# swami1995/SimuRLacra

Hardware: AMD Instinct MI355X
Metric: env-steps/sec whole node, 65 536 QQubeSwingUpSim envs, random policy (higher is better)
Workload: dtype f32

## Files before the change

scratch/ubench/rec_stream.hip:

```cpp
#include <hip/hip_runtime.h>
#include <cstdio>
#include <cstdlib>
typedef float v4f __attribute__((ext_vector_type(4)));
template <int LAYOUT, bool NT>
__global__ __launch_bounds__(256) void k(v4f* __restrict__ out, int n, int T, int pad, int jitter) {
    const int i = blockIdx.x * blockDim.x + threadIdx.x;
    const int wave = i >> 6, lane = i & 63;
    float x = (float)i * 1e-9f;
    const int mypad = pad + (jitter ? (wave * 2654435761u >> 16) % (unsigned)jitter : 0);
    for (int t = 0; t < T; ++t) {
        for (int q = 0; q < mypad; ++q) x = __builtin_fmaf(x, 0.999f, 1e-3f);
        v4f a = {x, x + 1.f, x + 2.f, x + 3.f}, b = {x + 4.f, x + 5.f, x + 6.f, x + 7.f};
        v4f *p0, *p1;
        if (LAYOUT == 0) {
            p0 = out + ((size_t)t * 2 + 0) * n + i;
            p1 = out + ((size_t)t * 2 + 1) * n + i;
        } else {
            p0 = out + (((size_t)wave * T + t) * 2 + 0) * 64 + lane;
            p1 = p0 + 64;
        }
        if (NT) {
            __builtin_nontemporal_store(a, p0);
            __builtin_nontemporal_store(b, p1);
        } else {
            *p0 = a;
            *p1 = b;
        }
    }
}
int main() {
    hipEvent_t e0, e1;
    hipEventCreate(&e0), hipEventCreate(&e1);
    const size_t cap = (size_t)6 << 30;
    v4f* buf;
    if (hipMalloc(&buf, cap) != hipSuccess) return 1;
    hipMemset(buf, 0, cap);
    const int ns[] = {65536, 131072, 262144, 1048576};
    const int pads[] = {0, 100, 200, 400};
    for (int n : ns)
        for (int wg : {64, 256})
            for (int pad : pads)
                for (int jit : {0, 64})
                    for (int layout = 0; layout < 2; ++layout)
                        for (int nt = 0; nt < 2; ++nt) {
                            size_t per_t = (size_t)n * 32;
                            int T = (int)((cap / 2) / per_t);
                            if (T > 400) T = 400;
                            float best = 1e30f;
                            for (int rep = 0; rep < 4; ++rep) {
                                v4f* o = buf + (rep & 1) * (cap / 2 / 16);
                                hipEventRecord(e0);
                                if (layout == 0 && nt == 0) k<0, false><<<n / wg, wg>>>(o, n, T, pad, jit);
                                if (layout == 0 && nt == 1) k<0, true><<<n / wg, wg>>>(o, n, T, pad, jit);
                                if (layout == 1 && nt == 0) k<1, false><<<n / wg, wg>>>(o, n, T, pad, jit);
                                if (layout == 1 && nt == 1) k<1, true><<<n / wg, wg>>>(o, n, T, pad, jit);
                                hipEventRecord(e1);
                                hipEventSynchronize(e1);
                                float ms;
                                hipEventElapsedTime(&ms, e0, e1);
                                if (rep && ms < best) best = ms;
                            }
                            printf("n=%8d wg=%3d pad=%3d jitter=%2d layout=%d nt=%d T=%3d : %7.1f us  %6.0f GB/s  %6.1f ns/step\n", n, wg, pad,
                                   jit, layout, nt, T, best * 1e3, per_t * T / best * 1e-6, best * 1e6 / T);
                            fflush(stdout);
                        }
    return 0;
}
```

simurlacra_amd/csrc/vecsim.hip:

```cpp
#include "vecsim_kernels.h"

namespace vs {

__global__ void k_bump_row(int* row) { *row += 1; }

__global__ __launch_bounds__(256) void k_rollout_lengths(const uint32_t* __restrict__ words, size_t ld, int n, int t_steps,
                                                         long long* __restrict__ lengths, uint8_t* __restrict__ done_last) {
    const int i = blockIdx.x * 256 + threadIdx.x;
    if (i >= n) return;
    const int nw = (t_steps + 31) / 32;
    int first = -1;
    for (int w = 0; w < nw && first < 0; ++w) {
        uint32_t bits = words[(size_t)w * ld + i];
        if (w == nw - 1 && (t_steps & 31)) bits &= (1u << (t_steps & 31)) - 1u;
        if (bits) first = w * 32 + (__ffs((int)bits) - 1);
    }
    lengths[i] = first < 0 ? (long long)t_steps : (long long)first + 1;
    done_last[i] = first >= 0;
}

__global__ void k_count_err(const uint8_t* err, int n, unsigned long long* out) {
    int i = blockIdx.x * BLOCK + threadIdx.x;
    bool e = i < n && err[i] != 0;
    unsigned long long m = __builtin_amdgcn_ballot_w64(e);
// ... 189 lines not shown
        out->s[q] = specs[q];
    }
    return VS_OK;
}

struct vs_mixed {
    int n = 0;
    vs_handle sub[MAX_SEG]{};
    Segs host{};
    Segs* dev = nullptr;
    int total_blocks = 0;
    std::string err;
};

static bool mixed_redraws(const vs_mixed* m) {
    for (int q = 0; q < m->n; ++q)
        if (m->sub[q]->d.dr_n > 0 || m->sub[q]->d.pbuf_n > 0) return true;
    return false;
}

static int mixed_upload(vs_mixed* m, const float* const* acts, const int64_t* env_strides, const int64_t* dim_strides,
                        int k_steps) {
    int blocks = 0;
    vs_handle h0 = m->sub[0];
    for (int q = 0; q < m->n; ++q) {
        vs_handle h = m->sub[q];
        if (h->d.pipe.act_on || h->d.pipe.obs_on) {
            m->err = "mixed batch: a segment carries an action/observation pipeline (single-family handles only)";
            return VS_ERR_STATE;
        }
        Seg& sg = m->host.s[q];
        blocks += (h->d.ld + BLOCK - 1) / BLOCK;
        sg.type = h->type;
        sg.block_end = blocks;
        sg.T = h->task;
        sg.d = h->d;
        sg.act = acts ? acts[q] : nullptr;
        sg.env_stride = env_strides ? (long)env_strides[q] : 0;
        sg.dim_stride = dim_strides ? (long)dim_strides[q] : 0;
        sg.reset_seed = h->ar_seed;
        sg.epoch0 = h->epoch;
        h->epoch += (uint64_t)k_steps;
    }
    m->host.n = m->n;
    m->total_blocks = blocks;
    hipError_t e = hipMemcpyAsync(m->dev, &m->host, sizeof(Segs), hipMemcpyHostToDevice, h0->stream);
    if (e == hipSuccess) e = hipStreamSynchronize(h0->stream);
    if (e != hipSuccess) { m->err = std::string("mixed_upload: ") + hipGetErrorString(e); return VS_ERR_HIP; }
    return VS_OK;
}

extern "C" {

int vs_version(void) { return 304; }

static int record_width(int t, int mode) {
    const EnvInfo& e = ENV_INFO[t];
    return mode == 2 ? e.O + e.A + 1 + e.S + e.A + e.H : e.O + e.A + 1;
}

int vs_traj_layout(int t, int mode, int* F, int* nq, int* h2, int* h1) {
    if (t < 0 || t >= VS_ENV_COUNT || mode < 1 || mode > 2) return VS_ERR_ARG;
    const int f = record_width(t, mode);
    if (F) *F = f;
    if (nq) *nq = f / 4;
    if (h2) *h2 = (f % 4) >= 2 ? 1 : 0;
    if (h1) *h1 = f % 2;
    return VS_OK;
}

int vs_env_dims(int t, int* S, int* A, int* O, int* P, int* H, int* I, int* K) {
    if (t < 0 || t >= VS_ENV_COUNT) return VS_ERR_ARG;
    const EnvInfo& e = ENV_INFO[t];
    if (S) *S = e.S;
    if (A) *A = e.A;
    if (O) *O = e.O;
    if (P) *P = e.P;
    if (H) *H = e.H;
    if (I) *I = e.I;
    if (K) *K = e.K;
    return VS_OK;
}

const char* vs_env_name(int t) { return (t < 0 || t >= VS_ENV_COUNT) ? nullptr : ENV_INFO[t].name; }

const char* vs_param_name(int t, int i) {
    if (t < 0 || t >= VS_ENV_COUNT || i < 0 || i >= ENV_INFO[t].P) return nullptr;
    return ENV_INFO[t].pnames[i];
}

int vs_nominal_params(int t, int flags, float* out) {
    if (t < 0 || t >= VS_ENV_COUNT || !out) return VS_ERR_ARG;
    for (int k = 0; k < ENV_INFO[t].P; ++k) out[k] = ENV_INFO[t].nominal[k];
    if ((t == VS_ENV_QCP_SU || t == VS_ENV_QCP_ST) && (flags & VS_FLAG_LONG_POLE)) {
        out[12] = 0.23f;
        out[13] = 0.641f / 2;
    }
    return VS_OK;
}

const char* vs_last_error(vs_handle h) { return h ? h->err.c_str() : g_create_err.c_str(); }

int vs_create(int env_type, int64_t n_envs, double dt, int64_t max_steps, int device_id, const vs_task_cfg* cfg,
              vs_handle* out) {
    if (!out) return fail(nullptr, VS_ERR_ARG, "vs_create: out is NULL");
    *out = nullptr;
    if (env_type < 0 || env_type >= VS_ENV_COUNT) return fail(nullptr, VS_ERR_ARG, "vs_create: unknown env_type");
// ... 840 lines not shown
```

simurlacra_amd/csrc/vecsim_envs.h:

```cpp
#pragma once
#include <hip/hip_runtime.h>
#include <stdint.h>

#include <type_traits>

#include "vecsim_dual.h"

namespace vs {

constexpr int MAXS = 8, MAXA = 2, MAXO = 8, MAXH = 2, MAXP = 20, MAXK = 20;
constexpr double PI_D = 3.14159265358979323846;
constexpr float PI_F = (float)PI_D;
constexpr float PI_4_F = (float)(PI_D / 4.0), PI4_F = (float)(4.0 * PI_D), PI5_F = (float)(5.0 * PI_D),
                PI20_F = (float)(20.0 * PI_D), QQ_TH_MAX_F = (float)(115.0 / 180.0 * PI_D);
constexpr float TWO_PI_F = 6.28318530717958647692f;
constexpr float TWO_PI_HI = 6.28318548202514648437500f;
constexpr float TWO_PI_LO = -1.74845553146951715461910e-07f;

enum RewKind { REW_QUADR = 0, REW_EXP = 1, REW_SCALED_EXP = 2 };

struct Task {
    float des[MAXS];
    float qd[MAXS];
    float rd[MAXA];
// ... 135 lines not shown
        }
        return c;
    }
    __device__ __forceinline__ static uint4 philox(uint64_t seed, uint32_t env, uint32_t purpose, uint64_t t) {
        return rounds(make_uint4(env, purpose, (uint32_t)t, (uint32_t)(t >> 32)),
                      make_uint2((uint32_t)seed, (uint32_t)(seed >> 32)));
    }
    __device__ __forceinline__ static float to_u01(uint32_t bits) { return (float)(bits >> 8) * (1.0f / 16777216.0f); }
    __device__ __forceinline__ void block() {
        out = rounds(ctr, key);
        ctr.y += 0x10000u;
        used = 0;
    }
    __device__ __forceinline__ uint32_t next() {
        if (used == 4) block();
        uint32_t v = used == 0 ? out.x : used == 1 ? out.y : used == 2 ? out.z : out.w;
        ++used;
        return v;
    }
    __device__ __forceinline__ float u01() { return to_u01(next()); }
    __device__ __forceinline__ float uniform(float lo, float hi) { return lo + (hi - lo) * u01(); }
    __device__ __forceinline__ static void box_muller(uint32_t b0, uint32_t b1, float& z0, float& z1) {
        float u1 = 1.0f - to_u01(b0);
        float u2 = to_u01(b1);
        float r = __builtin_amdgcn_sqrtf(-1.3862944f * __builtin_amdgcn_logf(u1));
        z0 = r * __builtin_amdgcn_cosf(u2);
        z1 = r * __builtin_amdgcn_sinf(u2);
    }
    __device__ __forceinline__ float normal() {
        uint32_t b0 = next(), b1 = next();
        float z0, z1;
        box_muller(b0, b1, z0, z1);
        return z0;
    }
};
enum RngPurpose { RNG_ACT = 1, RNG_INIT = 2, RNG_PARAM = 3, RNG_ACT_NOISE = 4, RNG_OBS_NOISE = 5, RNG_POLICY_NOISE = 6 };

enum FinalKind { FINAL_NONE = 0, FINAL_CONST_MALUS = 1, FINAL_STATE_TIME = 2 };
template <int A_>
struct EnvDefaults {
    static constexpr bool SYMMETRIC_BOX = true;
    static constexpr int FINAL = FINAL_NONE;
    static constexpr bool WS_PAYS = true;
    static constexpr bool REWARD_SIDE_USES_CONSTS = true;
    static constexpr int WS_SHAPE_FULL = 64;
    static constexpr bool WS_MID = true;
    static constexpr int WS_MID_G3_FROM = 1 << 30;
    static constexpr int WS_SMALL = 64;
    static constexpr int WS_PREP_C = 0;
    static constexpr int WS_PREP_G64 = 0;
    static constexpr bool WS_DRAW_P = false;
    static constexpr bool WS_G3 = false;
    static constexpr int WS_G3_FULL = 256;
    static constexpr int WS_MIN_WAVES = 1;
    static constexpr bool WS_ALONE = false;
    template <class R>
    __device__ static void limit_act(const float*, const float* lo, const float* hi, const R* a_raw, R* a) {
#pragma unroll
        for (int j = 0; j < A_; ++j) {
            a[j] = vmin(vmax(a_raw[j], lo[j]), hi[j]);
            if (visnan(a_raw[j])) a[j] = a_raw[j];
        }
    }
    __device__ static float sample_action(const float*, float lo, float hi, float u01, int) { return lo + (hi - lo) * u01; }
    static constexpr int TRIG = 0, TRIG_AT = 0;
    template <class R>
    __device__ static void observe_p(const R*, R*) {}
};
#define VS_OBSERVE_C_IS_OBSERVE \
    template <class R>          \
    __device__ static void observe_c(const R* s, const R*, R* o) { observe(s, o); }

struct Omo : EnvDefaults<1> {
    static constexpr int WS_MID_G3_FROM = 0;
    static constexpr int WS_PREP_G64 = 1;
    static constexpr int S = 2, A = 1, O = 2, H = 0, I = 2, P = 3, K = 4, KS = 4;
    static constexpr int REW = REW_QUADR, RADIAL = -1, CMAX = -1;
    static constexpr int FINAL = FINAL_CONST_MALUS;
    static constexpr bool WS_DRAW_P = true;
    static constexpr bool WS_G3 = true;
    enum { C_A10, C_A11, C_B1, C_AMAX };
    __device__ static void calc_consts(const Task&, const float* p, float* c) {
        float m = p[0], k = p[1], d = p[2];
        float omega = sqrtf(k / m);
        float zeta = d / (2.0f * sqrtf(m * k));
        c[C_A10] = -(omega * omega);
        c[C_A11] = -2.0f * zeta * omega;
        c[C_B1] = 1.0f / m;
        c[C_AMAX] = 1.0f * k;
    }
    __device__ static void state_bounds(const float*, float* lo, float* hi) {
        hi[0] = 1.0f; hi[1] = 10.0f; lo[0] = -1.0f; lo[1] = -10.0f;
    }
    __device__ static void act_bounds(const float* c, float* lo, float* hi) { hi[0] = c[C_AMAX]; lo[0] = -c[C_AMAX]; }
    template <class R>
    __device__ static void dynamics(const Task& T, const float* c, R* s, R*, const R* a, const R*) {
        R sd0 = s[1];
        R sd1 = c[C_A10] * s[0] + c[C_A11] * s[1] + c[C_B1] * a[0];
        s[0] = s[0] + sd0 * T.dt;
        s[1] = s[1] + sd1 * T.dt;
    }
    template <class R>
    __device__ static void observe(const R* s, R* o) { o[0] = s[0]; o[1] = s[1]; }
    VS_OBSERVE_C_IS_OBSERVE
    __device__ static void sample_init(const Task&, const float*, Rng& g, float* init) {
        init[0] = g.uniform(-0.75f, -0.65f);
// ... 553 lines not shown
```

simurlacra_amd/csrc/vecsim_kernels.h:

```cpp
#pragma once
#include <hip/hip_runtime.h>

#include <climits>
#include <cmath>
#include <cstdio>
#include <cstdlib>
#include <cstring>
#include <new>
#include <string>
#include <type_traits>
#include <vector>

#include "../../include/vecsim.h"
#include "vecsim_envs.h"

namespace vs {

constexpr int BLOCK = 256;

struct DrSpecs {
    int n;
    vs_dp_spec s[MAXP];
};

// ... 689 lines not shown
            if (!UNI) E::act_bounds(c, alo, ahi);
        } else {
            if (fin) {
                es.count += 1u;
                es.retsum += ret;
                es.lensum += step;
            }
            if (d.log_episodes) append_episode(d, fin, i, ret, step);
            frozen |= done;
            if (!REC && __builtin_amdgcn_ballot_w64(!frozen) == 0ull) break;
        }
#ifdef VS_ABLATE_OBSERVE
        if (REC) { for (int j = 0; j < E::O; ++j) ob[j] = s[j % E::S]; }
#else
        if (REC) E::observe(s, ob);
#endif
    }
    i = VS_COLD(i);
    if (!REC) E::observe(s, ob);
    if (PIPE && d.pipe.obs_on) pipe_obs<E>(d, i, es.epi, step, ob, ob);
#pragma unroll
    for (int j = 0; j < E::S; ++j) d.state[j * ld + i] = s[j];
#pragma unroll
    for (int j = 0; j < E::H; ++j) d.hidden[j * ld + i] = h[j];
#pragma unroll
    for (int j = 0; j < E::O; ++j) d.obs[j * ld + i] = ob[j];
    d.step[i] = step;
    d.ret[i] = ret;
    d.rew[i] = rew;
    d.done[i] = done;
    d.failed[i] = failed;
    if (E::FINAL != FINAL_NONE) d.yielded[i] = yielded;
    d.ep_idx[i] = es.epi;
    d.es_count[i] = es.count;
    d.es_retsum[i] = es.retsum;
    d.es_lensum[i] = es.lensum;
}

template <class E, bool UNI, bool AR, int REC, bool PIPE, bool DRK = false>
__global__ __launch_bounds__(BLOCK) void k_rollout(Task T, Dev d, int k_steps, uint64_t seed, uint64_t reset_seed,
                                                   uint64_t epoch0) {
    rollout_body<E, UNI, AR, REC, PIPE, DRK>(T, d, k_steps, seed, reset_seed, epoch0, (int)blockIdx.x);
}

enum : unsigned { WSF_DONE = 1u, WSF_FAILED = 2u, WSF_FROZEN = 4u, WSF_FIN = 8u };

__device__ __forceinline__ void ws_barrier() {
#ifdef VS_WS_NOSYNC
    return;
#endif
    asm volatile("s_waitcnt lgkmcnt(0)\n\ts_barrier" ::: "memory");
}

constexpr int FNN_MAXH = 4;
constexpr int FNN_W = 64;
constexpr int FNN_XS = 12;
__host__ __device__ constexpr int fnn_waves(int n_hidden) { return n_hidden <= 2 ? 8 : 4; }
enum FnnNonlin { FNN_ID = 0, FNN_TANH = 1, FNN_RELU = 2, FNN_SIGMOID = 3 };
struct Fnn {
    const float* w;
    int n_hidden, in_dim, out_dim;
    int hidden[FNN_MAXH];
    int hid_nonlin[FNN_MAXH], out_nonlin;
    int feat;
    int n_vis;
    int obs_idx[MAXO];
    int ident;
    int noisy;
    float noise_std[MAXA];
    int off_w[FNN_MAXH + 1], off_b[FNN_MAXH + 1];
};

__device__ __forceinline__ float tanh_fast(float x) {
    float t = __builtin_amdgcn_exp2f(-2.885390081777927f * fabsf(x));
    float r = (1.0f - t) * rcp_fast(1.0f + t);
    return copysignf(r, x);
}
__device__ __forceinline__ float fnn_nonlin(int kind, float x) {
    if (kind == FNN_TANH) return tanh_fast(x);
    if (kind == FNN_RELU) return fmaxf(x, 0.f);
    if (kind == FNN_SIGMOID) return rcp_fast(1.0f + __builtin_amdgcn_exp2f(-1.4426950408889634f * x));
    return x;
}

__device__ __forceinline__ float wave_sum_to_lane63(float v) {
#define VS_DPP_ADD(ctrl, rmask)                                                                                             \
    v += __builtin_bit_cast(float, __builtin_amdgcn_update_dpp(0, __builtin_bit_cast(int, v), ctrl, rmask, 0xF, false))
    VS_DPP_ADD(0xB1, 0xF);
    VS_DPP_ADD(0x4E, 0xF);
    VS_DPP_ADD(0x141, 0xF);
    VS_DPP_ADD(0x140, 0xF);
    VS_DPP_ADD(0x142, 0xA);
    VS_DPP_ADD(0x143, 0xC);
#undef VS_DPP_ADD
    return v;
}

__device__ __forceinline__ void wave_lds_fence() {
    __builtin_amdgcn_fence(__ATOMIC_RELEASE, "wavefront");
    __builtin_amdgcn_wave_barrier();
    __builtin_amdgcn_fence(__ATOMIC_ACQUIRE, "wavefront");
}

typedef float fnn_acc __attribute__((ext_vector_type(16)));
template <class E, bool AR, int REC, int NHID, int NE, bool MF = false>
__global__ __launch_bounds__(64 * fnn_waves(NHID)) void k_rollout_fnn(Task T, Dev d, Fnn P, int k_steps, uint64_t reset_seed,
// ... 310 lines not shown
            auto_reset<E, UNI>(T, d, fin, i, reset_seed, c, s, h, step, ret, yielded, es);
            E::act_bounds(c, alo, ahi);
        } else {
            if (fin) {
                es.count += 1u;
                es.retsum += ret;
                es.lensum += step;
            }
            if (d.log_episodes) append_episode(d, fin, i, ret, step);
            frozen |= done;
        }
        E::observe(s, ob);
    }
    if (!envw) return;
#pragma unroll
    for (int j = 0; j < E::S; ++j) d.state[j * ld + i] = s[j];
#pragma unroll
    for (int j = 0; j < E::H; ++j) d.hidden[j * ld + i] = h[j];
#pragma unroll
    for (int j = 0; j < E::O; ++j) d.obs[j * ld + i] = ob[j];
    d.step[i] = step;
    d.ret[i] = ret;
    d.rew[i] = rew;
    d.done[i] = done;
    d.failed[i] = failed;
    if (E::FINAL != FINAL_NONE) d.yielded[i] = yielded;
    d.ep_idx[i] = es.epi;
    d.es_count[i] = es.count;
    d.es_retsum[i] = es.retsum;
    d.es_lensum[i] = es.lensum;
}

template <class E, bool UNI, bool AR, int REC, int WS_R, int NE, bool DP, int NR = 2, int DRK = 0>
__global__ __launch_bounds__(NR * NE)
__attribute__((amdgpu_waves_per_eu(NR == 3 ? 3 : E::WS_MIN_WAVES, (NE == 64 && NR == 2 && E::WS_ALONE) ? 1 : 0))) void k_rollout_ws(Task T, Dev d, int k_steps, uint64_t seed, uint64_t reset_seed,
                                                        uint64_t epoch0) {
    static_assert(DRK == 0 || (!UNI && AR), "a randomizer needs per-env constants and resets inside the launch");
    static_assert(DRK >= 0 && DRK <= 2, "none | randomizer | buffer");
    static_assert(E::FINAL != FINAL_STATE_TIME, "needs the post-step state on the reward side");
    static_assert(NE == 64 || NE == 128 || NE == 256, "envs per workgroup");
    static_assert(NR == 2 || (NR == 3 && !DP), "two roles, or three with the generator wave drawing the actions");
    constexpr bool G3 = NR == 3;
#ifdef VS_G_NOOBS
    constexpr bool GOBS = false;
#else
    constexpr bool GOBS = G3 && REC != 0 && E::O >= 4;
#endif
    constexpr int HM = REC == 2 ? E::H : 0;
    constexpr int AM = DP ? E::A : 0;
    constexpr int M0 = E::S + (REC ? E::TRIG : 0) + HM + AM + 1;
    constexpr int M = M0 % 4 == 3 ? M0 + 1 : M0;
    constexpr int TR0 = E::S, HM0 = E::S + (REC ? E::TRIG : 0), AM0 = HM0 + HM;
    constexpr int NT = E::TRIG > 0 ? E::TRIG : 1, NH = E::H > 0 ? E::H : 1;
    __shared__ __attribute__((aligned(16))) float l_msg[2][WS_R][M * NE];
#ifdef VS_PREP_G256
    constexpr int PCL = DP ? 0 : (E::WS_PREP_C > 0 ? E::WS_PREP_C : ((NR == 3 && DRK == 0) ? E::WS_PREP_G64 : 0));
#else
    constexpr int PCL = DP ? 0 : (E::WS_PREP_C > 0 ? E::WS_PREP_C : ((NR == 3 && NE == 64 && DRK == 0) ? E::WS_PREP_G64 : 0));
#endif
    constexpr bool PC = PCL > 0;
    static_assert(PCL != 2 || E::REWARD_SIDE_USES_CONSTS || DRK == 0, "a dead zone off the physics wave reads per-env constants: they must not change inside the launch");
    constexpr int AW = PC ? 2 * E::A : E::A;
    __shared__ __attribute__((aligned(16))) float l_act[G3 ? 3 : (DP ? 1 : 2)][DP ? 1 : WS_R][DP ? 4 : AW * NE];
    auto ab = [](int bb) __attribute__((always_inline)) { return DP ? 0 : (G3 ? bb % 3 : (bb & 1)); };
    constexpr bool STOCK = AR;
    constexpr int SKW = E::I + (REC ? E::TRIG : 0);
#ifdef VS_WS_REFILL
    constexpr int WS_REFILL = VS_WS_REFILL;
#else
    constexpr int WS_REFILL = 8;
#endif
    __shared__ float l_stock[STOCK ? SKW * NE : 1];
    __shared__ uint32_t l_stag[STOCK ? NE : 1];
    __shared__ uint32_t l_epi[(STOCK && G3) ? NE : 1];
    extern __shared__ float l_dyn[];
    const bool dr_stock = DRK == 1 ? (STOCK && !UNI && d.dr_n > 0) : (DRK == 2 && STOCK && !UNI && d.dr_n > 0 && d.pbuf_n == 0);
    const bool stock_on = STOCK && (DRK == 0 || (DRK == 1 ? true : (d.pbuf_n == 0 && (d.dr_n == 0 || dr_stock))));
    float* const l_npar = l_dyn;
    float* const l_ncon = l_dyn + E::P * NE;
    const int wave = threadIdx.x >> 6;
    const int role = wave / (NE / 64);
    const int le = threadIdx.x & (NE - 1);
    const int i = blockIdx.x * NE + le;
    const int le_ = le, i_ = i;
    const size_t ld = d.ld;
    const bool valid = i < d.n;
    const int nb = (k_steps + WS_R - 1) / WS_R;
    float c[E::K];
    load_consts<E, UNI>(d, i, c, 0, E::KS);
    float alo[E::A], ahi[E::A];
    E::act_bounds(c, alo, ahi);

    constexpr unsigned SPB = 4 / E::A;
    static_assert(WS_R % SPB == 0, "a batch is a whole number of Philox blocks");
    constexpr int NBLK = WS_R / SPB;
    const unsigned ph = (unsigned)(epoch0 % SPB);
    const uint64_t blk0 = epoch0 / SPB;
    uint4 carry = make_uint4(0, 0, 0, 0);
    auto draw_batch = [&](int bb, float (*a_out)[AW]) __attribute__((always_inline)) {
        uint32_t w[(NBLK + 1) * 4];
        w[0] = carry.x, w[1] = carry.y, w[2] = carry.z, w[3] = carry.w;
#pragma unroll
        for (int q = 1; q <= NBLK; ++q) {
            carry = Rng::philox(seed, d.idx0 + (uint32_t)i, RNG_ACT, blk0 + (uint64_t)bb * NBLK + (uint64_t)q);
            w[4 * q] = carry.x, w[4 * q + 1] = carry.y, w[4 * q + 2] = carry.z, w[4 * q + 3] = carry.w;
        }
#pragma unroll
        for (int r = 0; r < WS_R; ++r) {
#pragma unroll
            for (int j = 0; j < E::A; ++j) {
                uint32_t bits = w[r * E::A + j];
#pragma unroll
                for (unsigned p2 = 1; p2 < SPB; ++p2) bits = ph == p2 ? w[(r + p2) * E::A + j] : bits;
                bool nrm = (T.flags & VS_FLAG_ACT_NORM) != 0;
                a_out[r][(PC ? E::A : 0) + j] = E::sample_action(c, nrm ? -1.0f : alo[j], nrm ? 1.0f : ahi[j], Rng::to_u01(bits), j);
            }
            if constexpr (PC) {
                const float* a = a_out[r] + E::A;
                float an[E::A], ac[E::A];
                const bool nrm = (T.flags & VS_FLAG_ACT_NORM) != 0;
                float lb[E::A], ub[E::A];
                E::act_bounds(c, lb, ub);
#pragma unroll
                for (int j = 0; j < E::A; ++j) {
                    float m = lb[j] + (a[j] + 1.0f) * (ub[j] - lb[j]) * 0.5f;
                    an[j] = vsel(nrm, m, a[j]);
                }
                E::limit_act(c, alo, ahi, an, ac);
                if constexpr (PCL == 2) E::dead_zone(T, c, ac);
#pragma unroll
                for (int j = 0; j < E::A; ++j) a_out[r][j] = ac[j];
            }
        }
    };

    uint32_t c_epi = 0u;
    uint32_t c_tag = 0xFFFFFFFFu;
    auto refill = [&]() __attribute__((always_inline)) {
        if (!STOCK) return;
        if (G3) c_epi = __hip_atomic_load(&l_epi[le], __ATOMIC_RELAXED, __HIP_MEMORY_SCOPE_WORKGROUP);
        const bool need = stock_on && valid && c_tag != c_epi;
#ifdef VS_WS_REFILL_MIN
        constexpr int REFILL_MIN = DRK == 1 ? VS_WS_REFILL_MIN : 1;
#else
        constexpr int REFILL_MIN = DRK == 1 ? 8 : 1;
#endif
        if (__builtin_popcountll(__builtin_amdgcn_ballot_w64(need)) < REFILL_MIN) return;
        const int i = VS_COLD(i_), le = VS_COLD(le_);
        if (dr_stock) {
            Rng gp(reset_seed, d.idx0 + (uint32_t)i, RNG_PARAM, (uint64_t)c_epi);
            const int n = d.dr_n;
            for (int q = 0; q < n; ++q) {
                const vs_dp_spec sp = d.drv.s[q];
                const float v = draw_one_param(sp, gp);
                if (need) l_npar[sp.param_index * NE + le] = v;
            }
        }
        if (need) {
            float cs[E::K];
#pragma unroll
            for (int k = 0; k < E::K; ++k) cs[k] = k < E::KS ? c[k] : 0.f;
            if (dr_stock) {
                float p[E::P];
#pragma unroll
                for (int k = 0; k < E::P; ++k) p[k] = l_npar[k * NE + le];
                E::calc_consts(T, p, cs);
#pragma unroll
                for (int k = 0; k < E::K; ++k) l_ncon[k * NE + le] = cs[k];
            }
            Rng g(reset_seed, d.idx0 + (uint32_t)i, RNG_INIT, (uint64_t)c_epi);
            float init[E::I];
            E::sample_init(T, cs, g, init);
#pragma unroll
            for (int j = 0; j < E::I; ++j) l_stock[j * NE + le] = init[j];
            if (REC && E::TRIG > 0) {
                float s0[E::S], tr0[NT];
                E::state_from_init(init, s0);
                E::observe_p(s0, tr0);
#pragma unroll
                for (int j = 0; j < E::TRIG; ++j) l_stock[(E::I + j) * NE + le] = tr0[j];
            }
            __hip_atomic_store(&l_stag[le], c_epi, __ATOMIC_RELEASE, __HIP_MEMORY_SCOPE_WORKGROUP);
            c_tag = c_epi;
        }
    };
    auto draw = [&](int bb) __attribute__((always_inline)) {
        if (DP) return;
        float a_new[WS_R][AW];
        draw_batch(bb, a_new);
#pragma unroll
        for (int r = 0; r < WS_R; ++r) Planes<AW>::store(l_act[ab(bb)][DP ? 0 : r], NE, le, a_new[r]);
    };

    if (role == 0) {
        __builtin_amdgcn_s_setprio(3);
        float s[E::S], h[NH], tr[NT], ob[E::O];
#pragma unroll
        for (int j = 0; j < E::S; ++j) s[j] = d.state[j * ld + i];
#pragma unroll
        for (int j = 0; j < E::H; ++j) h[j] = d.hidden[j * ld + i];
        int step = d.step[i];
        uint32_t epi = d.ep_idx[i];
        bool frozen = !AR && d.done[i] != 0;
        bool done = d.done[i] != 0, failed = d.failed[i] != 0;
        bool err_acc = false;
        if (REC) E::observe_p(s, tr);
        if (DP) carry = Rng::philox(seed, d.idx0 + (uint32_t)i, RNG_ACT, blk0);
        __builtin_amdgcn_s_waitcnt(0x0F70);
        ws_barrier();
        auto p_step = [&](const float* a, float* msg) __attribute__((always_inline)) {
            {
                float v[M];
#pragma unroll
                for (int j = 0; j < E::S; ++j) v[j] = s[j];
                if (REC) {
#pragma unroll
                    for (int j = 0; j < E::TRIG; ++j) v[TR0 + j] = tr[j];
                }
#pragma unroll
                for (int j = 0; j < HM; ++j) v[HM0 + j] = h[j];
#pragma unroll
                for (int j = 0; j < AM; ++j) v[AM0 + j] = a[j];
                bool fin = false;
                if (!frozen) {
                    if constexpr (PCL == 2) {
                        E::dynamics_core(T, c, s, h, a, (REC && E::TRIG > 0) ? (const float*)tr : (const float*)nullptr);
                    } else if constexpr (PCL == 1) {
                        E::dynamics(T, c, s, h, a, (REC && E::TRIG > 0) ? (const float*)tr : (const float*)nullptr);
                    } else {
                        float an[E::A], ac[E::A];
                        {
                            const bool nrm = (T.flags & VS_FLAG_ACT_NORM) != 0;
                            float lb[E::A], ub[E::A];
                            E::act_bounds(c, lb, ub);
#pragma unroll
                            for (int j = 0; j < E::A; ++j) {
                                float m = lb[j] + (a[j] + 1.0f) * (ub[j] - lb[j]) * 0.5f;
                                an[j] = vsel(nrm, m, a[j]);
                            }
                        }
                        E::limit_act(c, alo, ahi, an, ac);
                        E::dynamics(T, c, s, h, ac, (REC && E::TRIG > 0) ? (const float*)tr : (const float*)nullptr);
// ... 24 lines not shown
#pragma unroll
                            for (int j = 0; j < E::S; ++j) err_acc |= isnan(s[j]);
                            load_consts<E, UNI>(d, i, c, E::KS, E::K);
                            bool stocked = false;
                            if (STOCK) {
                                const uint32_t tag = __hip_atomic_load(&l_stag[le], __ATOMIC_ACQUIRE, __HIP_MEMORY_SCOPE_WORKGROUP);
                                stocked = tag == epi;
                                if (stocked) {
                                    if (dr_stock) {
#pragma unroll
                                        for (int k = 0; k < E::K; ++k) c[k] = l_ncon[k * NE + le];
#pragma unroll
                                        for (int k = 0; k < E::P; ++k) d.params[(size_t)k * ld + i] = l_npar[k * NE + le];
#pragma unroll
                                        for (int k = 0; k < E::K; ++k) d.consts[(size_t)k * ld + i] = c[k];
                                    }
                                    float init[E::I];
#pragma unroll
                                    for (int j = 0; j < E::I; ++j) init[j] = l_stock[j * NE + le];
                                    if (REC) {
#pragma unroll
                                        for (int j = 0; j < E::TRIG; ++j) tr[j] = l_stock[(E::I + j) * NE + le];
                                    }
                                    E::state_from_init(init, s);
                                    E::init_hidden(T, c, nullptr, s, h, false);
                                }
                            }
#ifdef VS_WS_STAMP
                            if (d.dbg) atomicAdd(d.dbg + ((size_t)(i >> 6) * 3 + 0) * 4, stocked ? 1ull : (1ull << 32));
#endif
                            if (!stocked) {
                                reset_lane_sampled<E>(T, d, DRK != 0, i, reset_seed, (uint64_t)epi, c, s, h,
                                                      dr_stock ? (const float*)l_npar : (const float*)nullptr, NE, le, DRK == 2);
                                if (REC) E::observe_p(s, tr);
                            }
                            epi += 1u;
                            step = 0;
                            if (STOCK && G3) __hip_atomic_store(&l_epi[le], epi, __ATOMIC_RELEASE, __HIP_MEMORY_SCOPE_WORKGROUP);
                        }
                        if (!UNI) E::act_bounds(c, alo, ahi);
#ifdef VS_WS_STAMP
                        VS_STAMP(sr1);
                        if (d.dbg && (threadIdx.x & 63) == 0) {
                            atomicAdd(d.dbg + ((size_t)(i >> 6) * 3 + 2) * 4 + 0, sr1 - sr0);
                            atomicAdd(d.dbg + ((size_t)(i >> 6) * 3 + 2) * 4 + 1, 1ull);
                        }
#endif
                    }
                } else {
                    frozen |= done;
                }
            }
        };
        auto p_batch_full = [&](int b) __attribute__((always_inline)) {
            float a_all[WS_R][AW];
            if (DP) {
                draw_batch(b, a_all);
            } else {
#pragma unroll
                for (int r = 0; r < WS_R; ++r) Planes<AW>::load(l_act[ab(b)][DP ? 0 : r], NE, le, a_all[r]);
            }
#pragma unroll
            for (int r = 0; r < WS_R; ++r) p_step(a_all[r], l_msg[b & 1][r]);
        };
        auto p_batch_ragged = [&](int b, int nr) __attribute__((always_inline)) {
            float a_all[WS_R][AW];
            if (DP) draw_batch(b, a_all);
#pragma unroll 1
            for (int r = 0; r < nr; ++r) {
                float a[AW];
                if (DP) {
#pragma unroll
                    for (int j = 0; j < AW; ++j) {
                        a[j] = a_all[0][j];
#pragma unroll
                        for (int q = 1; q < WS_R; ++q) a[j] = r == q ? a_all[q][j] : a[j];
                    }
                } else {
                    Planes<AW>::load(l_act[ab(b)][DP ? 0 : r], NE, le, a);
                }
                p_step(a, l_msg[b & 1][r]);
            }
        };
#ifdef VS_WS_NOP
        for (int b = 0; b < nb; ++b) ws_barrier();
        if (false)
#endif
#ifdef VS_WS_STAMP
        unsigned long long acc0 = 0, acc1 = 0, acc2 = 0;
#endif
        for (int b = 0; b < nb; ++b) {
            const int nr = min(WS_R, k_steps - b * WS_R);
            VS_STAMP(st0);
            if (nr == WS_R) p_batch_full(b);
            else p_batch_ragged(b, nr);
            VS_STAMP(st2);
            ws_barrier();
#ifdef VS_WS_STAMP
            VS_STAMP(st3);
            acc1 += st2 - st0, acc2 += st3 - st2;
#endif
        }
#ifdef VS_WS_STAMP
        if ((threadIdx.x & 63) == 0 && d.dbg) {
            unsigned long long* q = d.dbg + ((size_t)(i >> 6) * 3 + 0) * 4;
            q[1] = acc1, q[2] = acc2, q[3] = (unsigned long long)nb;
        }
#endif
        const int i = VS_COLD(i_);
#pragma unroll
        for (int j = 0; j < E::S; ++j) err_acc |= isnan(s[j]);
        if (err_acc && valid) d.err[i] = 1;
        E::observe(s, ob);
#pragma unroll
        for (int j = 0; j < E::S; ++j) d.state[j * ld + i] = s[j];
#pragma unroll
        for (int j = 0; j < E::H; ++j) d.hidden[j * ld + i] = h[j];
#pragma unroll
        for (int j = 0; j < E::O; ++j) d.obs[j * ld + i] = ob[j];
        d.step[i] = step;
        d.ep_idx[i] = epi;
        d.done[i] = done;
        d.failed[i] = failed;
    } else if (role == 1) {
        const size_t rec0 = (size_t)d.traj_t0;
        float ret = d.ret[i];
        float rew = d.rew[i];
        bool yielded = E::FINAL != FINAL_NONE ? d.yielded[i] != 0 : false;
        EpStat es{0u, d.es_count[i], d.es_retsum[i], d.es_lensum[i]};
        int len = d.step[i];
        DoneBits db;
        if (REC) db.begin(d, i, rec0);
        if (STOCK && !G3) {
            c_epi = d.ep_idx[i];
            l_stag[le] = 0xFFFFFFFFu;
            if (dr_stock) {
#pragma unroll
                for (int k = 0; k < E::P; ++k) l_npar[k * NE + le] = d.params[(size_t)k * ld + i];
            }
        }
        if (!DP && !G3) carry = Rng::philox(seed, d.idx0 + (uint32_t)i, RNG_ACT, blk0);
        auto work_off = [&](auto full_tag, int bb, int nr) __attribute__((always_inline)) {
            constexpr bool FULL = decltype(full_tag)::value;
            float v[WS_R][M], a[WS_R][E::A], rw[WS_R], ob[WS_R][E::O], a_app[WS_R][E::A];
#pragma unroll
            for (int r = 0; r < WS_R; ++r) {
                if (!FULL && r >= nr) continue;
                Planes<M>::load(l_msg[bb & 1][r], NE, le, v[r]);
                if (DP) {
#pragma unroll
                    for (int j = 0; j < E::A; ++j) a[r][j] = v[r][AM0 + j];
                } else if (PC) {
                    float ua[AW];
                    Planes<AW>::load(l_act[ab(bb)][DP ? 0 : r], NE, le, ua);
#pragma unroll
                    for (int j = 0; j < E::A; ++j) a[r][j] = ua[E::A + j];
                } else {
                    Planes<E::A>::load(l_act[ab(bb)][DP ? 0 : r], NE, le, a[r]);
                }
            }
#pragma unroll
            for (int r = 0; r < WS_R; ++r) {
                if (!FULL && r >= nr) continue;
                float an[E::A];
                {
                    const bool nrm = (T.flags & VS_FLAG_ACT_NORM) != 0;
                    float lb[E::A], ub[E::A];
                    E::act_bounds(c, lb, ub);
#pragma unroll
                    for (int j = 0; j < E::A; ++j) {
                        float m = lb[j] + (a[r][j] + 1.0f) * (ub[j] - lb[j]) * 0.5f;
                        an[j] = vsel(nrm, m, a[r][j]);
                    }
                }
                rw[r] = step_reward<E, float>(T, c, v[r], an);
                if (REC) E::observe_c(v[r], v[r] + TR0, ob[r]);
                if (REC == 2) applied_action<E>(T, c, alo, ahi, a[r], a_app[r]);
            }
            bool dn[WS_R];
#pragma unroll
            for (int r = 0; r < WS_R; ++r) {
                if (!FULL && r >= nr) continue;
                const unsigned fl = __float_as_uint(v[r][M0 - 1]);
                const bool was_frozen = !AR ? (fl & WSF_FROZEN) != 0u : false;
                const bool done = (fl & WSF_DONE) != 0u, failed = (fl & WSF_FAILED) != 0u;
                const bool fin = done && !was_frozen && valid;
                dn[r] = done;
                if (!was_frozen) {
                    len += 1;
                    rew = rw[r];
                    if (E::FINAL == FINAL_CONST_MALUS) {
                        if (done && !yielded) {
                            if (failed) rew += -1000.0f;
                            yielded = true;
                        }
                    }
                    ret += rew;
                } else {
                    rew = 0.f;
                }
                rw[r] = rew;
                if (__builtin_amdgcn_ballot_w64(fin) != 0ull) {
                    if (d.log_episodes) append_episode(d, fin, i, ret, len);
                    if (fin) {
                        es.count += 1u;
                        es.retsum += ret;
                        es.lensum += len;
                        if (AR) {
                            ret = 0.f;
                            yielded = false;
                            len = 0;
                            c_epi += 1u;
                        }
                    }
                }
            }
            if (REC) {
#pragma unroll
                for (int r = 0; r < WS_R; ++r) {
                    if (!FULL && r >= nr) continue;
                    const int t = bb * WS_R + r;
                    store_record<E, REC, GOBS ? 1 : 0>(d.traj_rec + (rec0 + (size_t)t) * Rec<E, REC>::F * ld, ld, i, ob[r], a[r], rw[r],
                                                       v[r], a_app[r], v[r] + HM0);
                    db.put(d, i, rec0 + (size_t)t, dn[r], t == k_steps - 1);
                }
            }
        };
        auto work = [&](int bb) __attribute__((always_inline)) {
            const int nr = min(WS_R, k_steps - bb * WS_R);
            if (nr == WS_R) work_off(std::true_type{}, bb, nr);
            else work_off(std::false_type{}, bb, nr);
        };
        __builtin_amdgcn_s_waitcnt(0x0F70);
        if (!G3) draw(0);
        ws_barrier();
#ifdef VS_WS_NOC
        for (int b = 0; b < nb; ++b) ws_barrier();
        if (false)
#endif
#ifdef VS_WS_STAMP
        unsigned long long acc0 = 0, acc1 = 0, acc2 = 0;
#endif
        for (int b = 0; b < nb; ++b) {
            VS_STAMP(st0);
            if (b >= 1) work(b - 1);
            VS_STAMP(st1);
            if (!G3) {
                if (b + 1 < nb) draw(b + 1);
                if ((b & (WS_REFILL - 1)) == 0) refill();
            }
            VS_STAMP(st2);
            ws_barrier();
#ifdef VS_WS_STAMP
            VS_STAMP(st3);
            acc0 += st1 - st0, acc1 += st2 - st1, acc2 += st3 - st2;
#endif
        }
#ifdef VS_WS_STAMP
        if ((threadIdx.x & 63) == 0 && d.dbg) {
            unsigned long long* q = d.dbg + ((size_t)(i >> 6) * 3 + 1) * 4;
            q[0] = acc0, q[1] = acc1, q[2] = acc2, q[3] = (unsigned long long)nb;
        }
#endif
        work(nb - 1);
        const int i = VS_COLD(i_);
        d.ret[i] = ret;
        d.rew[i] = rew;
        if (E::FINAL != FINAL_NONE) d.yielded[i] = yielded;
        d.es_count[i] = es.count;
        d.es_retsum[i] = es.retsum;
        d.es_lensum[i] = es.lensum;
    } else {
        if constexpr (G3) {
            const size_t rec0 = (size_t)d.traj_t0;
            if (STOCK) {
                c_epi = d.ep_idx[i];
                l_stag[le] = 0xFFFFFFFFu;
                l_epi[le] = c_epi;
                if (dr_stock) {
#pragma unroll
                    for (int k = 0; k < E::P; ++k) l_npar[k * NE + le] = d.params[(size_t)k * ld + i];
                }
            }
            carry = Rng::philox(seed, d.idx0 + (uint32_t)i, RNG_ACT, blk0);
            auto obs_off = [&](auto full_tag, int bb, int nr) __attribute__((always_inline)) {
                constexpr bool FULL = decltype(full_tag)::value;
#pragma unroll
                for (int r = 0; r < WS_R; ++r) {
                    if (!FULL && r >= nr) continue;
                    float v[M], ob[E::O];
                    Planes<M>::load(l_msg[bb & 1][r], NE, le, v);
                    E::observe_c(v, v + TR0, ob);
                    const int t = bb * WS_R + r;
                    float* row = d.traj_rec + (rec0 + (size_t)t) * Rec<E, REC>::F * ld;
                    Planes<4>::template store<0, true>(row, ld, i, ob);
                }
            };
            auto obs_work = [&](int bb) __attribute__((always_inline)) {
                if (!GOBS) return;
                const int nr = min(WS_R, k_steps - bb * WS_R);
                if (nr == WS_R) obs_off(std::true_type{}, bb, nr);
                else obs_off(std::false_type{}, bb, nr);
            };
            __builtin_amdgcn_s_waitcnt(0x0F70);
            draw(0);
            ws_barrier();
#ifdef VS_WS_NOG
            for (int b = 0; b < nb; ++b) ws_barrier();
            if (false)
#endif
#ifdef VS_WS_STAMP
            unsigned long long acc0 = 0, acc1 = 0, acc2 = 0;
#endif
            for (int b = 0; b < nb; ++b) {
                VS_STAMP(st0);
                if (b + 1 < nb) draw(b + 1);
                if ((b & (WS_REFILL - 1)) == 0) refill();
                VS_STAMP(st1);
                if (b >= 1) obs_work(b - 1);
                VS_STAMP(st2);
                ws_barrier();
#ifdef VS_WS_STAMP
                VS_STAMP(st3);
                acc0 += st1 - st0, acc1 += st2 - st1, acc2 += st3 - st2;
#endif
            }
#ifdef VS_WS_STAMP
            if ((threadIdx.x & 63) == 0 && d.dbg) {
                unsigned long long* q = d.dbg + ((size_t)(i >> 6) * 3 + 2) * 4;
                q[0] = acc0, q[1] = acc1, q[2] = acc2, q[3] = (unsigned long long)nb;
            }
#endif
            obs_work(nb - 1);
        }
    }
}

constexpr int MAX_SEG = 5;
struct Seg {
    int type;
    int block_end;
    Task T;
    Dev d;
    const float* act;
    long env_stride, dim_stride;
    uint64_t reset_seed, epoch0;
};
struct Segs {
    int n;
    Seg s[MAX_SEG];
};

#ifdef VS_TU_MIXED
#define MIXED_DISPATCH(type, ...)                                 \
    switch (type) {                                               \
        case VS_ENV_OMO: { using E = Omo; __VA_ARGS__; } break;     \
        case VS_ENV_BOB: { using E = Bob; __VA_ARGS__; } break;     \
        case VS_ENV_QQ_SU: { using E = QQ; __VA_ARGS__; } break;    \
        case VS_ENV_QCP_SU: { using E = Qcp; __VA_ARGS__; } break;  \
        case VS_ENV_QBB: { using E = Qbb; __VA_ARGS__; } break;     \
        case VS_ENV_QQ_ST: { using E = QQSt; __VA_ARGS__; } break;  \
        case VS_ENV_QCP_ST: { using E = QcpSt; __VA_ARGS__; } break;\
        case VS_ENV_PEND: { using E = Pend; __VA_ARGS__; } break;   \
        default: { using E = BobD; __VA_ARGS__; } break;            \
    }

template <bool AR, int REC, bool DRK = false>
__global__ __launch_bounds__(BLOCK) void k_rollout_mixed(const Segs* __restrict__ segs, int k_steps, uint64_t seed) {
    int b = blockIdx.x, q = 0, first = 0;
    int n = segs->n;
    while (q < n - 1 && b >= segs->s[q].block_end) first = segs->s[q++].block_end;
    const Seg& sg = segs->s[q];
    MIXED_DISPATCH(sg.type, (rollout_body<E, false, AR, REC, false, DRK>(sg.T, sg.d, k_steps, seed, sg.reset_seed, sg.epoch0, b - first)));
}

template <bool AR, bool DRK = false>
__global__ __launch_bounds__(BLOCK) void k_step_mixed(const Segs* __restrict__ segs) {
    int b = blockIdx.x, q = 0, first = 0;
    int n = segs->n;
    while (q < n - 1 && b >= segs->s[q].block_end) first = segs->s[q++].block_end;
    const Seg& sg = segs->s[q];
    MIXED_DISPATCH(sg.type, (step_body<E, false, AR, false, 0, DRK>(sg.T, sg.d, sg.act, sg.env_stride, sg.dim_stride, sg.reset_seed, b - first)));
}
#endif

// ... 426 lines not shown
```

Baseline: 186.0 billion.

## Replace workgroup barriers with LDS counter handoff between warp-specialized roles

In the G3 warp-specialized rollout kernel, the per-batch s_barrier between the physics, consumer and generator waves is replaced with per-wave-group LDS counters that each role posts and polls. The message and action ring buffers deepen (up to 4 slots, sized to the LDS budget) so roles can run several batches apart instead of in lockstep. This targets the stall cost of full-workgroup barriers when role work is uneven. It adds spin-wait polling with s_sleep and more LDS use, which may cut occupancy, and relies on relaxed workgroup-scope atomics being ordered correctly. A microbenchmark head mode and a stamp-analysis script are also added.

```diff
diff --git a/scratch/ubench/rec_stream.hip b/scratch/ubench/rec_stream.hip
--- a/scratch/ubench/rec_stream.hip
+++ b/scratch/ubench/rec_stream.hip
@@ -1,6 +1,9 @@
 #include <hip/hip_runtime.h>
+#include <algorithm>
 #include <cstdio>
 #include <cstdlib>
+#include <cstring>
+#include <vector>
 typedef float v4f __attribute__((ext_vector_type(4)));
 template <int LAYOUT, bool NT>
 __global__ __launch_bounds__(256) void k(v4f* __restrict__ out, int n, int T, int pad, int jitter) {
@@ -28,7 +31,55 @@
         }
     }
 }
-int main() {
+__global__ __launch_bounds__(512) void k_head(v4f* __restrict__ rec, uint32_t* __restrict__ done, int n, int T) {
+    const int wave = threadIdx.x >> 6, lane = threadIdx.x & 63;
+    const int plane = wave >> 2;
+    const int i = blockIdx.x * 256 + (wave & 3) * 64 + lane;
+    float x = (float)i * 1e-9f;
+    uint32_t w = 0u;
+    for (int t = 0; t < T; ++t) {
+        x = __builtin_fmaf(x, 0.999f, 1e-3f);
+        v4f a = {x, x + 1.f, x + 2.f, x + 3.f};
+        __builtin_nontemporal_store(a, rec + ((size_t)t * 2 + plane) * n + i);
+        if (plane == 1) {
+            w |= (x > 0.5f ? 1u : 0u) << (t & 31);
+            if ((t & 31) == 31 || t == T - 1) {
+                done[(size_t)(t >> 5) * n + i] = w;
+                w = 0u;
+            }
+        }
+    }
+}
+static int head() {
+    const int n = 65536, T = 400, slots = 3, launches = 300, warm = 20;
+    const size_t per_launch = (size_t)T * 2 * n;
+    v4f* rec;
+    uint32_t* done;
+    if (hipMalloc(&rec, per_launch * slots * sizeof(v4f)) != hipSuccess) return 1;
+    if (hipMalloc(&done, (size_t)((T + 31) / 32) * n * slots * sizeof(uint32_t)) != hipSuccess) return 1;
+    hipMemset(rec, 0, per_launch * slots * sizeof(v4f));
+    std::vector<hipEvent_t> ev(launches + 1);
+    for (auto& e : ev) hipEventCreate(&e);
+    for (int l = 0; l < warm; ++l) k_head<<<n / 256, 512>>>(rec + (l % slots) * per_launch, done + (size_t)(l % slots) * 13 * n, n, T);
+    hipEventRecord(ev[0]);
+    for (int l = 0; l < launches; ++l) {
+        k_head<<<n / 256, 512>>>(rec + (l % slots) * per_launch, done + (size_t)(l % slots) * 13 * n, n, T);
+        hipEventRecord(ev[l + 1]);
+    }
+    hipEventSynchronize(ev[launches]);
+    std::vector<float> ms(launches);
+    for (int l = 0; l < launches; ++l) hipEventElapsedTime(&ms[l], ev[l], ev[l + 1]);
+    std::sort(ms.begin(), ms.end());
+    const double bytes = (double)n * T * 32.0 + (double)n * ((T + 31) / 32) * 4.0;
+    auto rate = [&](float m) { return bytes / (m * 1e-3) * 1e-12; };
+    printf("head: n=%d T=%d launches=%d (3 slots of %.0f MB)  median %.1f us (%.3f TB/s)  min %.1f us (%.3f TB/s)  p90 %.1f us\n", n, T,
+           launches, per_launch * 16 / 1e6, ms[launches / 2] * 1e3, rate(ms[launches / 2]), ms[0] * 1e3, rate(ms[0]), ms[launches * 9 / 10] * 1e3);
+    printf("head: bench.py's fused step moves 32.41 B per env step: ceiling %.3e env-steps/s at the median\n",
+           rate(ms[launches / 2]) * 1e12 / 32.41);
+    return 0;
+}
+int main(int argc, char** argv) {
+    if (argc > 1 && !strcmp(argv[1], "head")) return head();
     hipEvent_t e0, e1;
     hipEventCreate(&e0), hipEventCreate(&e1);
     const size_t cap = (size_t)6 << 30;
diff --git a/scratch/ws_stamps.py b/scratch/ws_stamps.py
--- /dev/null
+++ b/scratch/ws_stamps.py
@@ -0,0 +1,41 @@
+import ctypes as C
+import os
+import sys
+
+import numpy as np
+
+ROOT = os.path.dirname(os.path.dirname(os.path.abspath(__file__)))
+sys.path.insert(0, ROOT)
+import simurlacra_amd as vs
+from bench import ENV_KW
+
+CASES = [("qq-su", 65536, "k_rollout_ws256g", 1), ("qq-su", 65536, "k_rollout_ws64g", 1), ("qq-su", 65536, "k_rollout_ws64", 1),
+         ("qq-su", 65536, "k_rollout_ws256g", 0), ("qq-su", 4096, "k_rollout_ws64g", 1), ("omo", 65536, "k_rollout_ws256g", 1),
+         ("bob", 65536, "k_rollout_ws256g", 1), ("pend", 65536, "k_rollout_ws256g", 1), ("qcp-su", 65536, "k_rollout_ws256g", 1),
+         ("qbb", 32768, "k_rollout_ws64g", 1)]
+if len(sys.argv) > 1:
+    CASES = [c for c in CASES if c[0] in sys.argv[1:]]
+LABELS = {0: (None, "4 steps", "wait"), 1: ("work_off", "draw+refill", "wait"), 2: ("draw+refill", "obs_off", "wait")}
+for name, n, var, rec in CASES:
+    env = vs.VecSimEnv(name, n, **ENV_KW[name])
+    env.set_params(np.tile(vs.nominal_params(name), (n, 1)))
+    env.set_auto_reset(True, seed=1)
+    env.reset(seed=2)
+    env.set_rollout_variant(var)
+    if rec:
+        env.set_traj_capacity(500)
+    for _ in range(3):
+        env.step_random(100, seed=3, record=bool(rec))
+    env.sync()
+    ms = env.time_step_kernel(iters=10, k_steps=100, record=bool(rec))
+    buf = np.zeros((env.ld // 64, 3, 4), dtype=np.uint64)
+    env._check(env._lib.vs_copy_to_host(env._h, 99, buf.ctypes.data_as(C.c_void_p)), "dbg")
+    env.close()
+    nb = float(buf[0, 0, 3])
+    print(f"{name} n={n} {var} rec={rec}: {ms * 1e3:.1f} us per 100 steps")
+    for role in range(3 if var.endswith("g") else 2):
+        m = buf[:, role, :3].astype(np.float64).mean(axis=0) / nb
+        if role == 0:
+            m[0] = 0.0
+        print(f"   {'PCG'[role]}: " + ", ".join(f"{lab} {v:7.1f} cyc/batch" for lab, v in zip(LABELS[role], m) if lab)
+              + f"  (sum {m.sum():.0f} = {m.sum() / 4:.0f} per step)")
diff --git a/simurlacra_amd/csrc/vecsim.hip b/simurlacra_amd/csrc/vecsim.hip
--- a/simurlacra_amd/csrc/vecsim.hip
+++ b/simurlacra_amd/csrc/vecsim.hip
@@ -265,7 +265,7 @@
 
 extern "C" {
 
-int vs_version(void) { return 304; }
+int vs_version(void) { return 305; }
 
 static int record_width(int t, int mode) {
     const EnvInfo& e = ENV_INFO[t];
diff --git a/simurlacra_amd/csrc/vecsim_envs.h b/simurlacra_amd/csrc/vecsim_envs.h
--- a/simurlacra_amd/csrc/vecsim_envs.h
+++ b/simurlacra_amd/csrc/vecsim_envs.h
@@ -211,6 +211,7 @@
     static constexpr bool WS_DRAW_P = false;
     static constexpr bool WS_G3 = false;
     static constexpr int WS_G3_FULL = 256;
+    static constexpr bool WS_HANDOFF = true;
     static constexpr int WS_MIN_WAVES = 1;
     static constexpr bool WS_ALONE = false;
     template <class R>
diff --git a/simurlacra_amd/csrc/vecsim_kernels.h b/simurlacra_amd/csrc/vecsim_kernels.h
--- a/simurlacra_amd/csrc/vecsim_kernels.h
+++ b/simurlacra_amd/csrc/vecsim_kernels.h
@@ -765,6 +765,16 @@
     asm volatile("s_waitcnt lgkmcnt(0)\n\ts_barrier" ::: "memory");
 }
 
+__device__ __forceinline__ void ho_post(uint32_t* ctr, int v) {
+    asm volatile("s_waitcnt lgkmcnt(0)" ::: "memory");
+    __hip_atomic_store(ctr, (uint32_t)v, __ATOMIC_RELAXED, __HIP_MEMORY_SCOPE_WORKGROUP);
+}
+__device__ __forceinline__ void ho_wait(const uint32_t* ctr, int v) {
+    while ((int)__builtin_amdgcn_readfirstlane(__hip_atomic_load(ctr, __ATOMIC_RELAXED, __HIP_MEMORY_SCOPE_WORKGROUP)) < v)
+        __builtin_amdgcn_s_sleep(1);
+    asm volatile("" ::: "memory");
+}
+
 constexpr int FNN_MAXH = 4;
 constexpr int FNN_W = 64;
 constexpr int FNN_XS = 12;
@@ -1181,7 +1191,13 @@
     constexpr int M = M0 % 4 == 3 ? M0 + 1 : M0;
     constexpr int TR0 = E::S, HM0 = E::S + (REC ? E::TRIG : 0), AM0 = HM0 + HM;
     constexpr int NT = E::TRIG > 0 ? E::TRIG : 1, NH = E::H > 0 ? E::H : 1;
-    __shared__ __attribute__((aligned(16))) float l_msg[2][WS_R][M * NE];
+#if defined(VS_WS_NOHO) || defined(VS_WS_NOP) || defined(VS_WS_NOC) || defined(VS_WS_NOG) || defined(VS_WS_NOSYNC)
+    constexpr bool HO = false;
+#else
+    constexpr bool HO = G3 && E::WS_HANDOFF;
+#endif
+    enum { HO_MSG, HO_CDONE, HO_GDONE, HO_ACT };
+    __shared__ __attribute__((aligned(16))) uint32_t l_ho[HO ? NE / 64 : 1][4];
 #ifdef VS_PREP_G256
     constexpr int PCL = DP ? 0 : (E::WS_PREP_C > 0 ? E::WS_PREP_C : ((NR == 3 && DRK == 0) ? E::WS_PREP_G64 : 0));
 #else
@@ -1190,8 +1206,14 @@
     constexpr bool PC = PCL > 0;
     static_assert(PCL != 2 || E::REWARD_SIDE_USES_CONSTS || DRK == 0, "a dead zone off the physics wave reads per-env constants: they must not change inside the launch");
     constexpr int AW = PC ? 2 * E::A : E::A;
-    __shared__ __attribute__((aligned(16))) float l_act[G3 ? 3 : (DP ? 1 : 2)][DP ? 1 : WS_R][DP ? 4 : AW * NE];
-    auto ab = [](int bb) __attribute__((always_inline)) { return DP ? 0 : (G3 ? bb % 3 : (bb & 1)); };
+    constexpr long HO_LDS0 = (long)(E::I + E::TRIG + 3 + (DRK == 1 ? E::P + E::K : 0)) * NE * 4;
+    constexpr auto ho_fits = [](long rm) { return (rm * M + (rm + 1) * AW) * WS_R * NE * 4 + HO_LDS0 <= 163840L * NE / 256; };
+    constexpr int RM = !HO ? 2 : (ho_fits(4) ? 4 : (ho_fits(3) ? 3 : 2));
+    constexpr int RA = HO ? RM + 1 : (G3 ? 3 : (DP ? 1 : 2));
+    __shared__ __attribute__((aligned(16))) float l_msg[RM][WS_R][M * NE];
+    __shared__ __attribute__((aligned(16))) float l_act[RA][DP ? 1 : WS_R][DP ? 4 : AW * NE];
+    auto ab = [](int bb) __attribute__((always_inline)) { return DP ? 0 : (int)((unsigned)bb % RA); };
+    auto mb = [](int bb) __attribute__((always_inline)) { return (int)((unsigned)bb % RM); };
     constexpr bool STOCK = AR;
     constexpr int SKW = E::I + (REC ? E::TRIG : 0);
 #ifdef VS_WS_REFILL
@@ -1210,8 +1232,21 @@
     const int wave = threadIdx.x >> 6;
     const int role = wave / (NE / 64);
     const int le = threadIdx.x & (NE - 1);
+    const int tri = le >> 6;
     const int i = blockIdx.x * NE + le;
     const int le_ = le, i_ = i;
+#ifdef VS_WS_STAMP
+    unsigned long long acc_w0 = 0, acc_w1 = 0;
+#define HO_WAIT(acc, ctr, v)     \
+    do {                         \
+        VS_STAMP(w0_);           \
+        ho_wait(ctr, v);         \
+        VS_STAMP(w1_);           \
+        acc += w1_ - w0_;        \
+    } while (0)
+#else
+#define HO_WAIT(acc, ctr, v) ho_wait(ctr, v)
+#endif
     const size_t ld = d.ld;
     const bool valid = i < d.n;
     const int nb = (k_steps + WS_R - 1) / WS_R;
@@ -1317,6 +1352,7 @@
         if (DP) return;
         float a_new[WS_R][AW];
         draw_batch(bb, a_new);
+        if (HO && bb >= RA) HO_WAIT(acc_w0, &l_ho[tri][HO_CDONE], bb + 1 - RA);
 #pragma unroll
         for (int r = 0; r < WS_R; ++r) Planes<AW>::store(l_act[ab(bb)][DP ? 0 : r], NE, le, a_new[r]);
     };
@@ -1447,16 +1483,38 @@
                 }
             }
         };
+        auto p_wait = [&](int b) __attribute__((always_inline)) {
+            HO_WAIT(acc_w0, &l_ho[tri][HO_ACT], b + 1);
+            HO_WAIT(acc_w0, &l_ho[tri][HO_CDONE], b - RM + 1);
+            if (GOBS) HO_WAIT(acc_w0, &l_ho[tri][HO_GDONE], b - RM + 1);
+        };
         auto p_batch_full = [&](int b) __attribute__((always_inline)) {
             float a_all[WS_R][AW];
             if (DP) {
                 draw_batch(b, a_all);
             } else {
+                uint32_t f[3] = {0u, 0u, 0u};
+                if (HO) {
+                    f[0] = __hip_atomic_load(&l_ho[tri][HO_ACT], __ATOMIC_RELAXED, __HIP_MEMORY_SCOPE_WORKGROUP);
+                    f[1] = __hip_atomic_load(&l_ho[tri][HO_CDONE], __ATOMIC_RELAXED, __HIP_MEMORY_SCOPE_WORKGROUP);
+                    if (GOBS) f[2] = __hip_atomic_load(&l_ho[tri][HO_GDONE], __ATOMIC_RELAXED, __HIP_MEMORY_SCOPE_WORKGROUP);
+                    asm volatile("" ::: "memory");
+                }
 #pragma unroll
                 for (int r = 0; r < WS_R; ++r) Planes<AW>::load(l_act[ab(b)][DP ? 0 : r], NE, le, a_all[r]);
-            }
-#pragma unroll
-            for (int r = 0; r < WS_R; ++r) p_step(a_all[r], l_msg[b & 1][r]);
+                if (HO) {
+                    const bool ok = (int)__builtin_amdgcn_readfirstlane(f[0]) >= b + 1 &&
+                                    (int)__builtin_amdgcn_readfirstlane(f[1]) >= b - RM + 1 &&
+                                    (!GOBS || (int)__builtin_amdgcn_readfirstlane(f[2]) >= b - RM + 1);
+                    if (!ok) {
+                        p_wait(b);
+#pragma unroll
+                        for (int r = 0; r < WS_R; ++r) Planes<AW>::load(l_act[ab(b)][DP ? 0 : r], NE, le, a_all[r]);
+                    }
+                }
+            }
+#pragma unroll
+            for (int r = 0; r < WS_R; ++r) p_step(a_all[r], l_msg[mb(b)][r]);
         };
         auto p_batch_ragged = [&](int b, int nr) __attribute__((always_inline)) {
             float a_all[WS_R][AW];
@@ -1474,7 +1532,7 @@
                 } else {
                     Planes<AW>::load(l_act[ab(b)][DP ? 0 : r], NE, le, a);
                 }
-                p_step(a, l_msg[b & 1][r]);
+                p_step(a, l_msg[mb(b)][r]);
             }
         };
 #ifdef VS_WS_NOP
@@ -1487,10 +1545,15 @@
         for (int b = 0; b < nb; ++b) {
             const int nr = min(WS_R, k_steps - b * WS_R);
             VS_STAMP(st0);
-            if (nr == WS_R) p_batch_full(b);
-            else p_batch_ragged(b, nr);
+            if (nr == WS_R) {
+                p_batch_full(b);
+            } else {
+                if (HO) p_wait(b);
+                p_batch_ragged(b, nr);
+            }
             VS_STAMP(st2);
-            ws_barrier();
+            if (HO) ho_post(&l_ho[tri][HO_MSG], b + 1);
+            else ws_barrier();
 #ifdef VS_WS_STAMP
             VS_STAMP(st3);
             acc1 += st2 - st0, acc2 += st3 - st2;
@@ -1499,7 +1562,7 @@
 #ifdef VS_WS_STAMP
         if ((threadIdx.x & 63) == 0 && d.dbg) {
             unsigned long long* q = d.dbg + ((size_t)(i >> 6) * 3 + 0) * 4;
-            q[1] = acc1, q[2] = acc2, q[3] = (unsigned long long)nb;
+            q[1] = acc1 - acc_w0, q[2] = acc2 + acc_w0, q[3] = (unsigned long long)nb;
         }
 #endif
         const int i = VS_COLD(i_);
@@ -1541,7 +1604,7 @@
 #pragma unroll
             for (int r = 0; r < WS_R; ++r) {
                 if (!FULL && r >= nr) continue;
-                Planes<M>::load(l_msg[bb & 1][r], NE, le, v[r]);
+                Planes<M>::load(l_msg[mb(bb)][r], NE, le, v[r]);
                 if (DP) {
 #pragma unroll
                     for (int j = 0; j < E::A; ++j) a[r][j] = v[r][AM0 + j];
@@ -1636,6 +1699,21 @@
 #ifdef VS_WS_STAMP
         unsigned long long acc0 = 0, acc1 = 0, acc2 = 0;
 #endif
+        if constexpr (HO) {
+            for (int b = 0; b < nb; ++b) {
+                HO_WAIT(acc_w0, &l_ho[tri][HO_MSG], b + 1);
+                VS_STAMP(st0);
+                work(b);
+                ho_post(&l_ho[tri][HO_CDONE], b + 1);
+#ifdef VS_WS_STAMP
+                VS_STAMP(st1);
+                acc0 += st1 - st0;
+#endif
+            }
+#ifdef VS_WS_STAMP
+            acc2 = acc_w0;
+#endif
+        } else {
         for (int b = 0; b < nb; ++b) {
             VS_STAMP(st0);
             if (b >= 1) work(b - 1);
@@ -1651,13 +1729,14 @@
             acc0 += st1 - st0, acc1 += st2 - st1, acc2 += st3 - st2;
 #endif
         }
+        }
+        if (!HO) work(nb - 1);
 #ifdef VS_WS_STAMP
         if ((threadIdx.x & 63) == 0 && d.dbg) {
             unsigned long long* q = d.dbg + ((size_t)(i >> 6) * 3 + 1) * 4;
             q[0] = acc0, q[1] = acc1, q[2] = acc2, q[3] = (unsigned long long)nb;
         }
 #endif
-        work(nb - 1);
         const int i = VS_COLD(i_);
         d.ret[i] = ret;
         d.rew[i] = rew;
@@ -1684,7 +1763,7 @@
                 for (int r = 0; r < WS_R; ++r) {
                     if (!FULL && r >= nr) continue;
                     float v[M], ob[E::O];
-                    Planes<M>::load(l_msg[bb & 1][r], NE, le, v);
+                    Planes<M>::load(l_msg[mb(bb)][r], NE, le, v);
                     E::observe_c(v, v + TR0, ob);
                     const int t = bb * WS_R + r;
                     float* row = d.traj_rec + (rec0 + (size_t)t) * Rec<E, REC>::F * ld;
@@ -1699,6 +1778,10 @@
             };
             __builtin_amdgcn_s_waitcnt(0x0F70);
             draw(0);
+            if (HO && (threadIdx.x & 63) == 0) {
+                l_ho[tri][HO_MSG] = 0u, l_ho[tri][HO_CDONE] = 0u, l_ho[tri][HO_GDONE] = 0u;
+                l_ho[tri][HO_ACT] = 1u;
+            }
             ws_barrier();
 #ifdef VS_WS_NOG
             for (int b = 0; b < nb; ++b) ws_barrier();
@@ -1709,12 +1792,19 @@
 #endif
             for (int b = 0; b < nb; ++b) {
                 VS_STAMP(st0);
-                if (b + 1 < nb) draw(b + 1);
+                if (b + 1 < nb) {
+                    draw(b + 1);
+                    if (HO) ho_post(&l_ho[tri][HO_ACT], b + 2);
+                }
                 if ((b & (WS_REFILL - 1)) == 0) refill();
                 VS_STAMP(st1);
-                if (b >= 1) obs_work(b - 1);
+                if (b >= 1 && GOBS) {
+                    if (HO) HO_WAIT(acc_w1, &l_ho[tri][HO_MSG], b);
+                    obs_work(b - 1);
+                    if (HO) ho_post(&l_ho[tri][HO_GDONE], b);
+                }
                 VS_STAMP(st2);
-                ws_barrier();
+                if (!HO) ws_barrier();
 #ifdef VS_WS_STAMP
                 VS_STAMP(st3);
                 acc0 += st1 - st0, acc1 += st2 - st1, acc2 += st3 - st2;
@@ -1723,9 +1813,10 @@
 #ifdef VS_WS_STAMP
             if ((threadIdx.x & 63) == 0 && d.dbg) {
                 unsigned long long* q = d.dbg + ((size_t)(i >> 6) * 3 + 2) * 4;
-                q[0] = acc0, q[1] = acc1, q[2] = acc2, q[3] = (unsigned long long)nb;
-            }
-#endif
+                q[0] = acc0 - acc_w0, q[1] = acc1 - acc_w1, q[2] = acc2 + acc_w0 + acc_w1, q[3] = (unsigned long long)nb;
+            }
+#endif
+            if (HO && GOBS && nb > 0) HO_WAIT(acc_w1, &l_ho[tri][HO_MSG], nb);
             obs_work(nb - 1);
         }
     }
```

Result: slower. 176.3 billion, median of 2 (-5.2%).
